# swishersnaaake/sexy-raytracer

Hardware: AMD Instinct MI355X
Metric: Msamples/s (WxHxspp/s), 720p masterchief @5k spp (higher is better)
Workload: dtype f32; 1 GPU; masterchief_720p_5000spp; scene=masterchief, width=1280, height=720, spp=5000, max_bounce=4, seed=1, spp_chunks=625, tree=reference, traversal=faithful (bvh.h order), parallelism=tiles8x8 interleaved over 1 rank(s), 1 gather (none)

## Files before the change

sexy-raytracer_amd/csrc/srt_api.cpp:

```cpp

#include <hip/hip_runtime.h>

#include <algorithm>
#include <cstdarg>
#include <cstdio>
#include <cstdlib>
#include <cstring>
#include <string>
#include <vector>

#include "srt_context.h"
#include "srt_launch.h"
#include "srt_thread.h"

int fail(SrtContext* ctx, const char* fmt, ...) {
  char buf[512];
  va_list ap;
  va_start(ap, fmt);
  vsnprintf(buf, sizeof buf, fmt, ap);
  va_end(ap);
  if (ctx) ctx->error = buf;
  fprintf(stderr, "srt_hip: %s\n", buf);
  return 1;
}

int wfCheck(SrtContext* ctx) {
  if (ctx->dWfError && *(volatile int32_t*)ctx->dWfError != 0) {
// ... 39 lines not shown
    {"node_burst", "SRT_NODE_BURST", &Tunables::nodeBurst, -1},
    {"ploc_radius", "SRT_PLOC_RADIUS", &Tunables::plocRadius, 64},
    {"fast_div", "SRT_FAST_DIV", &Tunables::fastDiv, 1},
    {"prim_again_min", "SRT_PRIM_AGAIN_MIN", &Tunables::primAgainMin, 4},
    {"keep_eighths", "SRT_KEEP_EIGHTHS", &Tunables::keepEighths, -1},
    {"chunk_scratch_mb", "SRT_CHUNK_SCRATCH_MB", &Tunables::chunkScratchMb, 12288},
    {"lds_tree", "SRT_LDS_TREE", &Tunables::ldsTree, 1},
    {"wavefront", "SRT_WAVEFRONT", &Tunables::wavefront, 256},
    {"wf_pool", "SRT_WF_POOL", &Tunables::wfPool, 2048},
    {"wf_swap_min", "SRT_WF_SWAP_MIN", &Tunables::wfSwapMin, 0},
    {"wf_swap_big", "SRT_WF_SWAP_BIG", &Tunables::wfSwapBig, 32},
    {"wf_profile", "SRT_WF_PROFILE", &Tunables::wfProfile, 0},
    {"wf_hybrid", "SRT_WF_HYBRID", &Tunables::wfHybrid, 1},
    {"wf_resident_max", "SRT_WF_RESIDENT_MAX", &Tunables::wfResidentMax, 0},
    {"wf_far_rounds", "SRT_WF_FAR_ROUNDS", &Tunables::wfFarRounds, 0},
    {"denoise_lds_step", "SRT_DENOISE_LDS_STEP", &Tunables::denoiseLdsStep, 4},
    {"tri_cert", "SRT_TRI_CERT", &Tunables::triCert, 1},
};

float triWMaxFor(const SrtContext* ctx) { return ctx->tun.triCert ? SRT_TRI_W_MAX : 0.0f; }

}

int checkSceneReady(SrtContext* ctx, const char* what) {
  if (!ctx->upload.haveScene) return fail(ctx, "%s: no scene uploaded", what);
  if (ctx->upload.geometryDirty) return fail(ctx, "%s: geometry was updated; call srtRefitScene before anything traverses the scene", what);
  return 0;
}

int buildDeviceTrees(SrtContext* ctx) {
// ... 19 lines not shown
  return 0;
}

static int srtUploadSceneImpl(SrtContext* ctx, const SrtSceneDesc* d) {
  if (!ctx || !d) return 1;
  HIP_OK(ctx, hipSetDevice(ctx->device));
  ctx->upload = Upload();
  ctx->temporalValid = false;
  std::string err = validateScene(d);
  HostScene h;
  if (err.empty()) err = flattenScene(d, SceneOptions{ctx->tun.wfHybrid, ctx->tun.wfResidentMax, ctx->tun.fastDiv}, h);
  if (!err.empty()) return fail(ctx, "%s", err.c_str());

  DevScene& s = ctx->upload.scene;
  if (!h.nodeThread.empty() && uploadVec(ctx, h.nodeThread, &s.nodeThread)) return 1;
  if (!h.nodesWf.empty() && (uploadVec(ctx, h.nodesWf, &s.nodesWf) || uploadVec(ctx, h.worldWf, &s.worldWf) || uploadVec(ctx, h.primSecond, &s.primSecond))) return 1;
  if (uploadVec(ctx, h.primClass, &s.primClass, 16) || uploadVec(ctx, h.nodeAxis, &s.nodeAxis, 64) || uploadVec(ctx, h.nodes, &s.nodes) ||
      uploadVec(ctx, h.triTest, &s.triTest) || uploadVec(ctx, h.triFast, &s.triFast) || uploadVec(ctx, h.triShade, &s.triShade) || uploadVec(ctx, h.spheres, &s.spheres) ||
      uploadVec(ctx, h.triPrimId, &s.triPrimId) || uploadVec(ctx, h.sphPrimId, &s.sphPrimId) || uploadVec(ctx, h.world, &s.world) ||
      uploadVec(ctx, h.materials, &s.materials) || uploadVec(ctx, h.shadeRecs, &s.shadeRecs) || uploadVec(ctx, h.textures, &s.textures) ||
      uploadVec(ctx, h.texels, &s.texels, 64))
    return 1;
  s.wfResident = h.wfResident;
  s.numPrimClass = (int32_t)h.primClass.size();
  s.numWorld = (int32_t)h.world.size();
  s.stackDepth = h.stackDepth;
  s.numNodes = (int32_t)(h.nodes.size() / 2);
  s.numTris = d->numTriangles;
  s.numSpheres = d->numSpheres;
  s.numMaterials = d->numMaterials;
// ... 226 lines not shown

int srtTestHybridRecords(const float* nodes8, int32_t numNodes, const int32_t* world, int32_t numWorld, int32_t numTriangles, int32_t numSpheres,
                         int32_t cap, float* outNodes8, int32_t* outWorld, int32_t* outSecond) {
  if (!nodes8 || !world || !outNodes8 || !outWorld || !outSecond || numNodes < 0 || numWorld < 0 || cap < 0) return -1;
  std::vector<float4> nodes(2 * (size_t)numNodes), wf;
  if (numNodes) memcpy(nodes.data(), nodes8, nodes.size() * sizeof(float4));
  std::vector<int32_t> w, second;
  const int32_t resident = srtHybridRecords(nodes, std::vector<int32_t>(world, world + numWorld), numTriangles, numSpheres, (size_t)cap, wf, w, second);
  if (resident <= 0) return 0;
  memcpy(outNodes8, wf.data(), wf.size() * sizeof(float4));
  memcpy(outWorld, w.data(), w.size() * sizeof(int32_t));
  memcpy(outSecond, second.data(), second.size() * sizeof(int32_t));
  return resident;
}

int srtTestGetTreeAux(SrtContext* ctx, int32_t item, uint8_t* outAxis, float* outPairs16, int32_t capacity, int32_t* count) {
  if (!ctx || !count) return 1;
  if (!ctx->upload.haveScene) return fail(ctx, "srtTestGetTreeAux: no scene uploaded");
  if (item < 0 || item >= (int32_t)ctx->upload.itemNodes.size()) return fail(ctx, "srtTestGetTreeAux: item %d out of range", item);
  HIP_OK(ctx, hipSetDevice(ctx->device));
  int32_t ref = 0;
  HIP_OK(ctx, hipMemcpy(&ref, ctx->upload.scene.world + item, sizeof ref, hipMemcpyDeviceToHost));
  if (ref < 0) return fail(ctx, "srtTestGetTreeAux: item %d is not a tree", item);
  const auto dt = std::find_if(ctx->upload.deviceBuilds.begin(), ctx->upload.deviceBuilds.end(), [&](const DeviceBuild& b) { return b.item == item; });
  const int32_t base = SRT_NODE_INDEX(ref), n = dt != ctx->upload.deviceBuilds.end() ? dt->count : (int32_t)ctx->upload.itemNodes[item].size();
  if (base + n > ctx->upload.scene.numNodes) return fail(ctx, "srtTestGetTreeAux: item %d lies outside the node array", item);
  *count = n;
  if (!outAxis && !outPairs16) return 0;
  if (capacity < n) return fail(ctx, "srtTestGetTreeAux: capacity %d < %d", capacity, n);
  if (outAxis) HIP_OK(ctx, hipMemcpy(outAxis, ctx->upload.scene.nodeAxis + base, (size_t)n, hipMemcpyDeviceToHost));
// ... 124 lines not shown
```

sexy-raytracer_amd/csrc/srt_context.h:

```cpp
#pragma once
#include <hip/hip_runtime.h>

#include <algorithm>
#include <cstring>
#include <exception>
#include <string>
#include <vector>

#include "srt_buffer.h"
#include "srt_device.h"
#include "srt_scene.h"

struct Tunables {
  int tileBlock, unitTiles, queues;
  int shadeMin, primMin, hitMin, fuseMin, nodeBurst;
  int plocRadius, fastDiv;
  int chunkScratchMb;
  int primAgainMin;
  int keepEighths;
  int ldsTree;
  int wavefront, wfPool, wfSwapMin, wfSwapBig, wfProfile;
  int wfHybrid, wfResidentMax, wfFarRounds;
  int denoiseLdsStep;
  int triCert;
};

struct Upload {
  std::vector<DeviceBuffer> sceneBuffers;
  DevScene scene{};
  bool haveScene = false;
  std::vector<std::vector<SrtBvhNode>> itemNodes;
  std::vector<DeviceBuild> deviceBuilds;
  std::vector<DeviceBuffer> buildRefs;
  int plocRadius = 0;
  int hostStackDepth = 0, hostBvhDepth = 0;
  std::vector<int32_t> hostTriPrimId, hostSphPrimId;
  int bvhDepth = 0;
  struct Tree {
    int32_t item, base, count;
    float time0, time1;
    bool deviceBuilt;
  };
  std::vector<Tree> trees;
  std::vector<int32_t> hostTriDevIndex, hostWfIndex;
  std::vector<uint8_t> itemBoxesStale;
  DeviceBuffer triDevIndex, wfIndex, refitUp, refitArrived;
  bool refitTables = false;
  bool refitLinksStale = false;
  bool geometryDirty = false;
  float pairTime0 = 0, pairTime1 = 0;
  int32_t fastDivOption = 0;
  DeviceBuffer prevTriTest, prevSpheres;
  bool haveSnapshot = false;
  bool epochSnapshot = false;
};

struct SrtContext {
  int device = 0;
  std::string error;
  Tunables tun{};
  hipDeviceProp_t prop;
// ... 117 lines not shown
```

sexy-raytracer_amd/csrc/srt_device.h:

```cpp
#ifndef SRT_DEVICE_H
#define SRT_DEVICE_H

#include <stdint.h>

#include "../../include/srt_hip.h"
#include "../../include/srt_hip_test.h"

#define SRT_REF_DONE ((int32_t)0x80000000)
#define SRT_NODE_REF(index) ((int32_t)(index) << 5)
#define SRT_NODE_INDEX(ref) ((int32_t)(ref) >> 5)
#define SRT_MAX_NODES (1 << 25)
#define SRT_MAX_QUEUES 64
#define SRT_BLOCK 256
#define SRT_BLOCK_TREE 1024
#define SRT_MAT_INDEX_MASK 0x00ffffff
#define SRT_MAT_TYPE_SHIFT 24
#define SRT_MAT_TEXTURED 4
#define SRT_MAT_FLAGS_SHIFT 28

struct DevMaterial {
  int32_t type;
  int32_t albedoTex, normalTex, metallicTex, roughnessTex;
  float albedo[4];
  float metalness, roughness;
// ... 27 lines not shown
  const int32_t* primSecond;
  int32_t wfResident;
  const int32_t* triPrimId;
  const int32_t* sphPrimId;
  const int32_t* world;
  int32_t numWorld;
  int32_t stackDepth;
  int32_t numNodes, numTris, numSpheres;
  int32_t fastDivScene;
  const DevMaterial* materials;
  const uint4* shadeRecs;
  int32_t numMaterials;
  const DevTexture* textures;
  const uint8_t* texels;
  int32_t texelBytes;
};

struct DevCamera {
  float origin[3], lleft[3], horizontal[3], vertical[3], hor[3], vert[3];
  float lensRadius, time0, time1;
};

struct SrtFixedAccum {
  long long r, g, b;
  uint32_t flags;
  uint32_t pad;
};

struct RenderArgs {
  DevScene scene;
// ... 205 lines not shown
```

sexy-raytracer_amd/csrc/srt_path.h:

```cpp
#ifndef SRT_PATH_H
#define SRT_PATH_H

#include <hip/hip_runtime.h>

#include <type_traits>
#include <stdint.h>

#include "srt_device.h"
#include "srt_slab.h"
#include "srt_tri_hit.h"

#define SRT_TREE_WAVES_PER_SIMD 4
#ifndef SRT_NODE_UNROLL
#define SRT_NODE_UNROLL 4
#endif
#ifndef SRT_NODE_UNROLL_CLOSEST
#define SRT_NODE_UNROLL_CLOSEST 4
#endif
#ifndef SRT_PRIM_ROUNDS
#define SRT_PRIM_ROUNDS 2
#endif
#ifndef SRT_RENDER_WAVES_PER_SIMD
#define SRT_RENDER_WAVES_PER_SIMD 5
#endif
// ... 118 lines not shown
  tMin = fmaxf(fminf(a, b), tMin);
  tMax = fminf(fmaxf(a, b), tMax);
  return !(tMax <= tMin);
}

__device__ __forceinline__ SrtSlab3 slab3(V3 v) { return SrtSlab3{v.x, v.y, v.z}; }
template <bool UNIFORM_TMIN>
__device__ __forceinline__ bool boxHitApprox(float4 n0, float4 n1, V3 r1, V3 m, float tolAbs, float tMin, float tMax,
                                             bool& undecided) {
  return srtSlabVerdict<UNIFORM_TMIN, false>(srtSlabEndsMinMax(n0, n1, slab3(r1), slab3(m)), tolAbs, tMin, tMax, undecided);
}
template <bool UNIFORM_TMIN>
__device__ __forceinline__ bool boxHitSign(float4 n0, float4 n1, V3 rp, V3 rq, V3 m, float tolAbs, float tMin, float tMax,
                                           bool& undecided) {
  return srtSlabVerdict<UNIFORM_TMIN, true>(srtSlabEndsSign(n0, n1, slab3(rp), slab3(rq), slab3(m)), tolAbs, tMin, tMax, undecided);
}
__device__ __forceinline__ bool boxMaybeHit(float4 lo, float4 hi, V3 r1, V3 m, float tolAbs, float tMin, float tMax, float& tEnter) {
  return srtSlabMaybe<false>(srtSlabEndsMinMax(lo, hi, slab3(r1), slab3(m)), tolAbs, tMin, tMax, tEnter);
}
__device__ __forceinline__ void slabSetup(const V3& o, const V3& r1, bool certified, V3& m, float& tolAbs) {
  SrtSlab3 mm;
  srtSlabSetup(slab3(o), slab3(r1), certified, mm, tolAbs);
  m = mk(mm.x, mm.y, mm.z);
}
__device__ __forceinline__ void slabSetupSign(const V3& o, const V3& r1, bool certified, V3& rp, V3& rq, V3& m, float& tolAbs) {
  SrtSlab3 p, q, mm;
  srtSlabSignSetup(slab3(o), slab3(r1), certified, p, q, mm, tolAbs);
  rp = mk(p.x, p.y, p.z);
  rq = mk(q.x, q.y, q.z);
  m = mk(mm.x, mm.y, mm.z);
// ... 498 lines not shown
```

sexy-raytracer_amd/csrc/srt_refit_host.cpp:

```cpp

#include <hip/hip_runtime.h>

#include <algorithm>
#include <cstdint>
#include <cstring>
#include <vector>

#include "srt_context.h"
#include "srt_launch.h"

namespace {

int checkUpdate(SrtContext* ctx, const char* what, int32_t first, int32_t count, int32_t have, const void* in, size_t align) {
  if (!ctx->upload.haveScene) return fail(ctx, "%s: no scene uploaded", what);
  if (first < 0 || count < 0 || (int64_t)first + count > have)
    return fail(ctx, "%s: range [%d, %d + %d) lies outside the scene's %d records", what, first, first, count, have);
  if (count == 0) return 2;
  if (!in) return fail(ctx, "%s: null records", what);
  if ((uintptr_t)in % align) return fail(ctx, "%s: records must be aligned to %zu bytes", what, align);
  return 0;
}

int triangleTable(SrtContext* ctx, const int32_t** out) {
  *out = nullptr;
// ... 92 lines not shown
    if (!ctx->upload.refitTables) {
      HIP_OK(ctx, ctx->upload.refitUp.reserve((size_t)n * sizeof(int32_t)));
      HIP_OK(ctx, ctx->upload.refitArrived.reserve((size_t)n * sizeof(int32_t)));
      HIP_OK(ctx, ctx->refitFlag.reserve(16));
      if (s.nodesWf) {
        if (ctx->upload.hostWfIndex.size() != (size_t)n) return fail(ctx, "%s: the hybrid records have no renumbering", what);
        HIP_OK(ctx, ctx->upload.wfIndex.reserve((size_t)n * sizeof(int32_t)));
        HIP_OK(ctx, hipMemcpy(ctx->upload.wfIndex.get(), ctx->upload.hostWfIndex.data(), (size_t)n * sizeof(int32_t), hipMemcpyHostToDevice));
      }
      ctx->upload.refitTables = ctx->upload.refitLinksStale = true;
    }
    if (ctx->upload.refitLinksStale) {
      const int e = srt_launch_refit_links(s.nodes, n, ctx->upload.refitUp.get<int32_t>(), stream);
      if (e) return fail(ctx, "%s: launch failed: %s", what, hipGetErrorString((hipError_t)e));
      ctx->upload.refitLinksStale = false;
    }
    HIP_OK(ctx, hipMemsetAsync(ctx->upload.refitArrived.get(), 0, (size_t)n * sizeof(int32_t), stream));
    HIP_OK(ctx, hipMemsetAsync(ctx->refitFlag.get(), 0, 16, stream));
    int e = 0;
    for (const Upload::Tree& t : ctx->upload.trees) {
      if (t.base < 0 || t.count < 1 || t.base + t.count > n) return fail(ctx, "%s: world item %d lies outside the node array", what, t.item);
      e = srt_launch_refit_nodes(&s, t.base, t.count, t.time0, t.time1, ctx->upload.refitUp.get<const int32_t>(), ctx->upload.refitArrived.get<int32_t>(),
                                 ctx->refitFlag.get<int32_t>(), t.deviceBuilt ? 1 : 0, stream);
      if (e) break;
    }
    if (!e) e = srt_launch_refit_derived(&s, s.nodesWf ? ctx->upload.wfIndex.get<const int32_t>() : nullptr, ctx->refitFlag.get<int32_t>(), stream);
    if (!e) e = srt_pair_nodes_async(&s, ctx->upload.pairTime0, ctx->upload.pairTime1, const_cast<float4*>(s.nodes2), stream);
    if (e) return fail(ctx, "%s: launch failed: %s", what, hipGetErrorString((hipError_t)e));
    HIP_OK(ctx, hipMemcpyAsync(&flag, ctx->refitFlag.get(), sizeof flag, hipMemcpyDeviceToHost, stream));
  }
  if (hipStreamSynchronize(stream) != hipSuccess) return fail(ctx, "%s: kernel failed: %s", what, hipGetErrorString(hipGetLastError()));
  ctx->upload.scene.fastDivScene = (flag & 3) == 0 ? ctx->upload.fastDivOption : 0;
  ctx->upload.scene.boxOrderedScene = (flag & 4) == 0 ? 1 : 0;
  if (ctx->motionTracking) {
    if (ctx->temporalRefits < 2) ctx->temporalRefits++;
    ctx->upload.epochSnapshot = false;
  } else {
    ctx->temporalValid = false;
  }
// ... 63 lines not shown
```

sexy-raytracer_amd/csrc/srt_render.cpp:

```cpp

#include <hip/hip_runtime.h>

#include <algorithm>
#include <cstring>
#include <vector>

#include "srt_context.h"
#include "srt_launch.h"

namespace {

size_t ldsBytesFor(const SrtContext* ctx, int maxBounce, int stackDepth) {
  return (size_t)(stackDepth + 2 + 3 * maxBounce + 3) * SRT_BLOCK * sizeof(int32_t) + 4 * sizeof(int32_t);
}

float chunkFixLimit(int32_t chunks) {
  int pow2 = 1;
  while (pow2 < chunks) pow2 *= 2;
  return 0x1p26f / (float)pow2;
}

}

extern "C" {
// ... 163 lines not shown
      if (!scratchPath) return fail(ctx, "render: cannot allocate %zu B for the pixel sums", need);
      scratchPath = false;
      HIP_OK(ctx, ctx->chunkScratch.reserve(planes * tilePixels * sizeof(SrtFixedAccum)));
    }
    if (scratchPath) {
      a.out = ctx->chunkScratch.get<float4>();
      a.chunkStride = (int32_t)tilePixels;
      if (moments) a.mout = a.out + tilePixels * a.sppChunks;
    } else {
      a.fix = ctx->chunkScratch.get<SrtFixedAccum>();
      if (moments) a.mfix = a.fix + tilePixels;
      HIP_OK(ctx, hipMemsetAsync(a.fix, 0, planes * tilePixels * sizeof(SrtFixedAccum), stream));
    }
  }
  const RenderPlan plan = renderPlan(ctx, p, moments, dList ? listTiles : -1);
  if (plan.lds > 160 * 1024) return fail(ctx, "render: BVH depth %d needs %zu B of LDS per workgroup", ctx->upload.scene.stackDepth, plan.lds);
  const RenderKernel kernel = plan.form >= 3 ? srt_render_wf_kernel_for(&plan) : srt_render_kernel_for(&plan);
  if (plan.lds > 64 * 1024)
    HIP_OK(ctx, hipFuncSetAttribute(reinterpret_cast<const void*>(kernel), hipFuncAttributeMaxDynamicSharedMemorySize, (int)plan.lds));
  int perCU = 1;
  if (plan.form < 3 && (hipOccupancyMaxActiveBlocksPerMultiprocessor(&perCU, kernel, plan.block, plan.lds) != hipSuccess || perCU < 1)) perCU = 1;
  const int wgItems = SRT_TILE_PIXELS * (plan.block / 64);
  int grid = std::min(ctx->prop.multiProcessorCount * perCU, (a.numWork + wgItems - 1) / wgItems);
  if (grid < 1) grid = 1;
  if (plan.form >= 3) {
    const int64_t itemsPerGroup = ((int64_t)a.numWork + grid - 1) / grid;
    const int wfPoolSize = (int)std::max<int64_t>(64, std::min<int64_t>(plan.wfRingCap, itemsPerGroup + 63));
    HIP_OK(ctx, ctx->wfPool.reserve((size_t)grid * wfPoolSize * 128));
    const int hiLevels = std::max(0, p->maxBounce - 4);
    HIP_OK(ctx, ctx->wfAttHi.reserve(std::max<size_t>(16, (size_t)grid * 3 * hiLevels * wfPoolSize * sizeof(float))));
// ... 541 lines not shown
```

sexy-raytracer_amd/csrc/srt_scene.cpp:

```cpp

#include "srt_scene.h"

#include <algorithm>
#include <cmath>
#include <cstdarg>
#include <cstdio>
#include <cstring>
#include <limits>
#include <random>

#include "srt_thread.h"

namespace {

std::mt19937& hostGenerator() {
  static std::mt19937 generator;
  return generator;
}
float hostRandomFloat() {
  static std::uniform_real_distribution<float> distribution(0.0f, 1.0f);
  return distribution(hostGenerator());
}
int hostRandomInt(int lo, int hi) {
  float a = (float)lo, b = (float)(hi + 1);
  return static_cast<int>(a + (b - a) * hostRandomFloat());
// ... 188 lines not shown
                    &h.triFast[SRT_TRI_FAST_SLOTS * (size_t)i]);
  }
  h.spheres.resize((size_t)d->numSpheres * 3);
  for (int i = 0; i < d->numSpheres; ++i) {
    const SrtSphereIn& s = d->spheres[i];
    sphereRecords(vec3(s.center0), vec3(s.center1), s.time0, s.time1, s.radius, s.material, &h.spheres[3 * (size_t)i]);
  }
  std::vector<int32_t> triDevIndex;
  auto devRef = [&](int32_t listRef) -> int32_t {
    const SrtPrimRef& p = d->prims[~listRef];
    if (p.type == SRT_PRIM_SPHERE) return ~((p.index << 1) | 1);
    return ~((triDevIndex.empty() ? p.index : triDevIndex[p.index]) << 1);
  };

  h.itemNodes.resize(d->numWorld);
  for (int w = 0; w < d->numWorld; ++w) {
    const SrtWorldItem& it = d->world[w];
    if (it.kind == SRT_WORLD_PRIM) {
      h.world.push_back(devRef(~it.first));
      continue;
    }
    if (!it.nodes && (it.builder == SRT_BUILDER_LBVH || it.builder == SRT_BUILDER_PLOC)) {
      int32_t base = (int32_t)(h.nodes.size() / 2), cnt = std::max(it.count - 1, 1);
      h.nodes.resize(h.nodes.size() + 2 * (size_t)cnt, make_float4(0, 0, 0, 0));
      h.nodeAxis.resize(h.nodeAxis.size() + cnt, 3);
      h.deviceBuilds.push_back(DeviceBuild{w, base, cnt, it.builder, it.time0, it.time1, {}});
      h.world.push_back(SRT_NODE_REF(base));
      continue;
    }
    Builder b;
    buildItem(d, it, b);
    int32_t base = (int32_t)(h.nodes.size() / 2);
// ... 180 lines not shown
    }
  }
  h.fastDivScene = certified ? o.fastDiv : 0;
  h.boxOrderedScene = ordered ? 1 : 0;
  if (h.deviceBuilds.empty() && !h.nodes.empty()) {
    srtThreadLinks16(h.nodes, h.world, d->numTriangles, d->numSpheres, h.nodeThread);
    if (o.wfHybrid > 0) {
      const size_t n = h.nodes.size() / 2;
      const size_t fits = (160 * 1024 - 64 * sizeof(int32_t) - 20 * 2048) / 32;
      const size_t fitsWhole = (160 * 1024 - 64 * sizeof(int32_t) - 18 * 1024) / 32;
      const size_t cap = o.wfResidentMax > 0 ? std::min<size_t>(fits, (size_t)o.wfResidentMax) : fits;
      if (n > (o.wfResidentMax > 0 ? cap : fitsWhole))
        h.wfResident = srtHybridRecords(h.nodes, h.world, d->numTriangles, d->numSpheres, cap, h.nodesWf, h.worldWf, h.primSecond, &h.wfIndex);
      if (h.nodesWf.empty()) h.wfIndex.clear();
    }
  }
  auto classOf = [&](float word, bool sphere) -> uint8_t {
    const int32_t bits = bitsAs<int32_t>(&word);
    const int type = (bits >> SRT_MAT_TYPE_SHIFT) & 3, flags = (bits >> SRT_MAT_FLAGS_SHIFT) & 3;
    if (type != SRT_MAT_PBR) return 2;
    if (!sphere) return 0;
    return flags ? 2 : 1;
  };
  h.triDevIndex.swap(triDevIndex);
  h.primClass.assign((size_t)2 * std::max(d->numTriangles, d->numSpheres) + 2, 2);
  for (int i = 0; i < d->numTriangles; ++i) h.primClass[(size_t)i << 1] = classOf(h.triShade[4 * (size_t)i + 3].w, false);
  for (int i = 0; i < d->numSpheres; ++i) h.primClass[((size_t)i << 1) | 1] = classOf(h.spheres[3 * (size_t)i + 1].w, true);
  return std::string();
}

// ... 34 lines not shown
```

sexy-raytracer_amd/csrc/srt_scene.h:

```cpp
#pragma once
#include <hip/hip_runtime.h>

#include <cstdint>
#include <string>
#include <vector>

#include "srt_device.h"
#include "srt_records.h"

struct BuildNode {
  Box box;
  int32_t left, right;
  uint8_t axis = 3;
};

struct Builder {
  const SrtSceneDesc* d;
  float time0, time1;
  std::vector<float> sortKey;
  std::vector<int32_t> objects;
  std::vector<BuildNode> nodes;
  int maxPending = 0;

  Box childBox(int32_t ref) const;
// ... 25 lines not shown
  float time0, time1;
};

struct HostScene {
  std::vector<float4> nodes;
  std::vector<uint8_t> nodeAxis;
  std::vector<int32_t> world;
  std::vector<float4> triTest, triShade, triFast, spheres;
  std::vector<int32_t> triPrimId, sphPrimId;
  std::vector<DevMaterial> materials;
  std::vector<DevTexture> textures;
  std::vector<uint8_t> texels;
  std::vector<uint4> shadeRecs;
  std::vector<uint8_t> primClass;
  std::vector<int32_t> nodeThread;
  std::vector<float4> nodesWf;
  std::vector<int32_t> worldWf, primSecond;
  int32_t wfResident = 0;
  std::vector<std::vector<SrtBvhNode>> itemNodes;
  std::vector<DeviceBuild> deviceBuilds;
  std::vector<HostTree> hostTrees;
  std::vector<int32_t> triDevIndex;
  std::vector<int32_t> wfIndex;
  int stackDepth = 0, bvhDepth = 0;
  int32_t fastDivScene = 0;
  int32_t boxOrderedScene = 0;
};

std::string flattenScene(const SrtSceneDesc* d, const SceneOptions& o, HostScene& out);
```

sexy-raytracer_amd/csrc/srt_slab.h:

```cpp
#pragma once
#include <hip/hip_runtime.h>
#include <math.h>

#include "srt_device.h"

struct SrtSlab3 {
  float x, y, z;
};

#define SRT_SLAB_FN SRT_HD __forceinline__
#if defined(__HIP_DEVICE_COMPILE__)
#define SRT_SLAB_ASM2(op, a, b)          \
  float r;                               \
  asm(op " %0, %1, %2" : "=v"(r) : "v"(a), "v"(b)); \
  return r
#define SRT_SLAB_ASM3(op, a, b, c)       \
  float r;                               \
  asm(op " %0, %1, %2, %3" : "=v"(r) : "v"(a), "v"(b), "v"(c)); \
  return r
#endif
SRT_SLAB_FN float srtSlabMin(float a, float b) {
#if defined(__HIP_DEVICE_COMPILE__)
  SRT_SLAB_ASM2("v_min_f32", a, b);
#else
// ... 78 lines not shown
  return srtSlabMin3(srtSlabMax(e.a.x, e.b.x), srtSlabMax(e.a.y, e.b.y), srtSlabMax(e.a.z, e.b.z));
}

#define SRT_SLAB_EPS 0x1p-21f

template <bool UNIFORM_TMIN, bool ORDERED>
SRT_SLAB_FN bool srtSlabVerdict(const SrtSlabEnds& e, float tolAbs, float tMin, float tMax, bool& undecided) {
  const float lo = srtSlabNear<ORDERED>(e);
  tMin = UNIFORM_TMIN ? srtSlabMaxUniform(lo, tMin) : srtSlabMax(lo, tMin);
  tMax = srtSlabMin(srtSlabFar<ORDERED>(e), tMax);
  const float diff = tMax - tMin;
  const float tol = __builtin_fmaf(SRT_SLAB_EPS, fabsf(tMax) + fabsf(tMin), tolAbs);
  undecided = !(fabsf(diff) > tol);
  return diff > tol;
}
template <bool ORDERED>
SRT_SLAB_FN bool srtSlabMaybe(const SrtSlabEnds& e, float tolAbs, float tMin, float tMax, float& tEnter) {
  const float t0 = srtSlabMax(srtSlabNear<ORDERED>(e), tMin);
  const float t1 = srtSlabMin(srtSlabFar<ORDERED>(e), tMax);
  const float tol = __builtin_fmaf(SRT_SLAB_EPS, fabsf(t1) + fabsf(t0), tolAbs);
  tEnter = t0;
  return !(t1 - t0 < -tol);
}
```

sexy-raytracer_amd/csrc/srt_wavefront.hip:

```cpp
#include "srt_path.h"
#include "srt_launch.h"
#include "srt_wf_links.h"
#include "srt_wf_rings.h"

#define WF_BLOCK 1024
#define WF_SET_OF(mask) std::integral_constant<uint32_t, (mask)>()
#define WF_CTX_BYTES 128
#define WF_CTL_LIVE 28
#define WF_CTL_ABORT 29
#define WF_CTL_WORDS 64
#define WF_PEND_MISS 0
#define WF_PEND_TERMINAL 2

namespace {
enum { W_NODE = 0, W_PRIM = 1, W_SWAP = 2, W_SERVE = 3 };

__device__ __forceinline__ void bufStore4(Rsrc r, int off, float4 v) {
  u32x4 u;
  u.x = __float_as_uint(v.x); u.y = __float_as_uint(v.y); u.z = __float_as_uint(v.z); u.w = __float_as_uint(v.w);
  __builtin_amdgcn_raw_buffer_store_b128(u, r, off, 0, 0);
}
__device__ __forceinline__ void bufStore1(Rsrc r, int off, uint32_t v) { __builtin_amdgcn_raw_buffer_store_b32(v, r, off, 0, 0); }
typedef float f32x4 __attribute__((ext_vector_type(4)));
typedef __attribute__((address_space(3))) const f32x4 LdsVec4;
// ... 10 lines not shown
  typedef typename std::conditional<HYBRID, int32_t, uint16_t>::type PrimSlot;
  extern __shared__ int32_t lds[];
  const DevScene& sc = a.scene;
  char* const ldsTree = reinterpret_cast<char*>(lds);
  const int resident = HYBRID ? sc.wfResident : sc.numNodes;
  const int treeBytes = resident * 32;
  int32_t* const ctl = reinterpret_cast<int32_t*>(ldsTree + treeBytes);
  const int RCAP = a.wfRingCap, POOL = a.wfPoolSize;
  uint16_t* const ringSlots = reinterpret_cast<uint16_t*>(ctl + WF_CTL_WORDS);
  float* const hitT = reinterpret_cast<float*>(ringSlots + WF_RINGS * RCAP);
  PrimSlot* const hitPrim = reinterpret_cast<PrimSlot*>(hitT + POOL);
  const int lane = threadIdx.x & 63;
  const unsigned long long laneBelow = (1ull << lane) - 1ull;
  const uint64_t seedMixed = mix64(a.seed);
  const V3 background = ld3(a.background);
  const Rsrc rsNodes = makeRsrc(HYBRID ? sc.nodesWf : sc.nodes, sc.numNodes * 32);
  const Rsrc rsTris = makeRsrc(sc.triTest, HYBRID ? sc.numTris * 48 : 0);
  const Rsrc rsFast = makeRsrc(sc.triFast, HYBRID ? 0 : sc.numTris * 64);
  const Rsrc rsSpheres = makeRsrc(sc.spheres, sc.numSpheres * 48);
  const Rsrc rsTexels = makeRsrc(sc.texels, sc.texelBytes);
  const Rsrc rsClass = makeRsrc(sc.primClass, sc.numPrimClass);
  const Rsrc rsSecond = makeRsrc(sc.primSecond, HYBRID ? sc.numPrimClass * 4 : 0);
  const Rsrc rsPool = makeRsrc(a.wfPool + (size_t)blockIdx.x * POOL * WF_CTX_BYTES, POOL * WF_CTX_BYTES);
  const int hiLevels = a.maxBounce > 4 ? a.maxBounce - 4 : 0;
  const Rsrc rsAttHi = makeRsrc(a.wfAttHi + (size_t)blockIdx.x * 3 * hiLevels * POOL, 3 * hiLevels * POOL * 4);
  const bool singleRoot = SINGLE || sc.numWorld == 1;
  auto worldRef = [&](int k) {
    if (HYBRID) return sc.worldWf[k];
    return srtWfRootWord(sc.world[k]);
  };
  const SrtWfRingGeom ringGeom = {a.wfRingCap, a.wfRingShift, a.wfRingMul3};

  {
    float4* dst = reinterpret_cast<float4*>(ldsTree);
    for (int i = threadIdx.x; i < resident * 2; i += WF_BLOCK) {
      float4 v = bufLoad4(rsNodes, 16 * i);
      if (!HYBRID) {
        const int32_t thread = sc.nodeThread[i >> 1];
        v.w = __int_as_float((i & 1) ? srtWfMissWord(thread) : srtWfHitWord(__float_as_int(v.w), thread));
      }
      dst[i] = v;
    }
    for (int i = threadIdx.x; i < WF_CTL_WORDS; i += WF_BLOCK) ctl[i] = 0;
    for (int i = threadIdx.x; i < WF_RINGS * RCAP; i += WF_BLOCK) ringSlots[i] = 0;
    __syncthreads();
    for (int id = threadIdx.x; id < POOL; id += WF_BLOCK) ringSlots[WF_RING_NEWITEM * RCAP + id] = (uint16_t)(id + 1);
    if (threadIdx.x == 0) {
      ctl[WF_CTL_TAIL(WF_RING_NEWITEM)] = POOL;
      ctl[WF_CTL_LIVE] = POOL;
    }
    if (threadIdx.x < 16) ctl[threadIdx.x] = (int)(blockIdx.x % (unsigned)a.numQueues);
    __syncthreads();
  }
// ... 162 lines not shown
      }
      return nNodes;
  };
  auto nodeBurst = [&](int nNodes) -> int {
      const int keep = (nNodes * a.keepEighths) >> 3;
      int budget = a.nodeBurst, left;
      auto visit = [&](const float4 n0, const float4 n1) {
        bool undecided;
        bool hitBox = SIGNFORM ? boxHitSign<true>(n0, n1, rp, rq, negOR, slabTol, a.tMin, closest, undecided)
                               : boxHitApprox<true>(n0, n1, rp, negOR, slabTol, a.tMin, closest, undecided);
        if (PROFILE) {
          const unsigned long long mu = __ballot(undecided);
          pLanes[8] += __popcll(mu);
          pLanes[7] += mu != 0 ? 1 : 0;
        }
        if (undecided) hitBox = boxHit(n0, n1, ray, a.tMin, closest);
        if constexpr (COUNT) {
          cnt[2]++;
          if (hitBox) cnt[3]++;
        }
        link = __float_as_int(n1.w);
        cur = hitBox ? __float_as_int(n0.w) : (HYBRID ? link >> 2 : link);
        if (!SINGLE && !singleRoot && cur == DONE && ++w < sc.numWorld) {
          cur = worldRef(w);
          link = DONE_PAIR;
        }
      };
      auto nodeVisit = [&](bool mine) {
        const bool here = HYBRID ? mine && (uint32_t)cur < (uint32_t)resident : cur >= 0;
        if (PROFILE) {
          pRuns[0]++;
// ... 501 lines not shown
```

sexy-raytracer_amd/hipdev.py:

```python
import ctypes as C
import os

import numpy as np

from . import abi

_HERE = os.path.dirname(os.path.abspath(__file__))
LIB_PATH = os.path.join(_HERE, "csrc", "libsrt_hip.so")
if os.environ.get("SRT_HIP_LIB"):
    LIB_PATH = os.path.abspath(os.environ["SRT_HIP_LIB"])

if not os.path.exists(LIB_PATH):
    raise ImportError("HIP extension not built: %s is missing (run __graft_entry__.build() or "
                      "`make -C sexy-raytracer_amd/csrc`)" % LIB_PATH)

try:
    import torch
except ImportError:
    pass

lib = C.CDLL(LIB_PATH)

EXPORTS = ["srtCreate", "srtDestroy", "srtLastError", "srtMakeCamera", "srtHostRandomFloat", "srtHostRandomReset",
           "srtUploadScene", "srtSetCamera", "srtBuildBvh", "srtGetBvh", "srtGetBvhDepth", "srtNumTiles", "srtNumLocalTiles", "srtDefaultSppChunks", "srtPlanSppChunks",
# ... 4 lines not shown
           "srtRenderTilesMoments", "srtRenderImageMoments", "srtDenoiseMoments", "srtRenderDenoisedImageMoments",
           "srtRenderAdaptive", "srtRenderAdaptiveImage",
           "srtTemporalAccumulate", "srtRenderTemporalFrame", "srtTemporalReset",
           "srtTemporalReproject", "srtRenderTemporalAdaptive", "srtRenderTemporalAdaptiveFrame",
           "srtRenderFeatureTileList", "srtRenderAdaptiveGuided", "srtRenderAdaptiveDenoisedImage",
           "srtRenderTemporalAdaptiveGuided", "srtRenderTemporalAdaptiveGuidedFrame",
           "srtUpdateTriangles", "srtUpdateSpheres", "srtUpdateTrianglesDevice", "srtUpdateSpheresDevice", "srtRefitScene",
           "srtRebuildScene", "srtGetTreeCost",
           "srtSetMotionTracking", "srtRenderMotionTiles", "srtRenderMotionImage", "srtTemporalAccumulateMotion",
           "srtTemporalReprojectMotion",
           "srtCommGetUniqueId", "srtCommInit", "srtGatherTiles", "srtRenderImageRanks", "srtCommDestroy",
           "srtLastKernelMs", "srtGetStats", "srtDeviceInfo"]
TEST_EXPORTS = ["srtSetTunable", "srtGetTunable", "srtGetShadeProfile", "srtGetWfProfile", "srtGetLaunchInfo", "srtRenderAov",
                "srtScatterRaysForm", "srtTestThreadLinks16", "srtTestHybridRecords", "srtTestGetTreeAux", "srtTestChunkSum",
                "srtTestDenoiseScratch", "srtTestGetTriUndecided", "srtTestGetTriFast", "srtTestTriFastRecord", "srtTestGetSlabScene",
                "srtTestRefinedRcp", "srtTestSlabVisit"]

_vp = C.c_void_p
lib.srtCreate.argtypes = [C.c_int, C.POINTER(_vp)]
lib.srtDestroy.argtypes = [_vp]
lib.srtLastError.argtypes = [_vp]
lib.srtLastError.restype = C.c_char_p
lib.srtMakeCamera.argtypes = [C.POINTER(abi.SrtCameraParams), C.POINTER(abi.SrtCamera)]
lib.srtHostRandomFloat.restype = C.c_float
lib.srtHostRandomReset.restype = None
lib.srtUploadScene.argtypes = [_vp, C.POINTER(abi.SrtSceneDesc)]
lib.srtSetCamera.argtypes = [_vp, C.POINTER(abi.SrtCamera)]
lib.srtBuildBvh.argtypes = [C.POINTER(abi.SrtSceneDesc), C.c_int32, _vp, C.c_int32, C.POINTER(C.c_int32),
                            C.POINTER(C.c_int32)]
lib.srtGetBvh.argtypes = [_vp, C.c_int32, _vp, C.c_int32, C.POINTER(C.c_int32)]
lib.srtGetBvhDepth.argtypes = [_vp, C.POINTER(C.c_int32)]
# ... 87 lines not shown
lib.srtGetWfProfile.argtypes = [_vp, _vp]
lib.srtGetLaunchInfo.argtypes = [_vp, _vp]
lib.srtTestThreadLinks16.argtypes = [_vp, C.c_int32, _vp, C.c_int32, C.c_int32, C.c_int32, _vp]
lib.srtTestHybridRecords.argtypes = [_vp, C.c_int32, _vp, C.c_int32, C.c_int32, C.c_int32, C.c_int32, _vp, _vp, _vp]
lib.srtTestThreadLinks16.restype = lib.srtTestHybridRecords.restype = C.c_int32
lib.srtTestGetTreeAux.argtypes = [_vp, C.c_int32, C.POINTER(C.c_uint8), C.POINTER(C.c_float), C.c_int32, C.POINTER(C.c_int32)]
if hasattr(lib, "srtTestGetTriUndecided"):
    lib.srtTestGetTriUndecided.argtypes = [_vp, C.POINTER(C.c_uint64)]
    lib.srtTestGetTriFast.argtypes = [_vp, _vp, C.c_int32, C.POINTER(C.c_int32)]
    lib.srtTestTriFastRecord.argtypes = [_vp, _vp]
if hasattr(lib, "srtTestGetSlabScene"):
    lib.srtTestGetSlabScene.argtypes = [_vp, C.POINTER(C.c_int32)]
if hasattr(lib, "srtTestRefinedRcp"):
    lib.srtTestRefinedRcp.argtypes = [_vp, C.c_int64, C.c_int64, C.POINTER(C.c_uint64)]
    lib.srtTestSlabVisit.argtypes = [_vp, C.POINTER(C.c_float), C.c_int32, C.c_float, C.c_int32, C.POINTER(C.c_float)]
lib.srtRenderAov.argtypes = [_vp, C.POINTER(abi.SrtRenderParams), C.c_int32, _vp]
lib.srtLastKernelMs.argtypes = [_vp, C.POINTER(C.c_float)]
lib.srtGetStats.argtypes = [_vp, C.POINTER(abi.SrtStats)]
lib.srtDeviceInfo.argtypes = [_vp, C.c_char_p, C.c_int32, C.POINTER(C.c_int32), C.POINTER(C.c_int32)]


class SrtError(RuntimeError):
    pass


def make_camera(params):
    cam = abi.SrtCamera()
    if lib.srtMakeCamera(C.byref(params), C.byref(cam)):
        raise SrtError("srtMakeCamera failed")
    return cam

# ... 585 lines not shown
        return int(out.value)

    def tri_fast_records(self):
        n = C.c_int32(0)
        self._check(lib.srtTestGetTriFast(self.h, None, 0, C.byref(n)))
        out = np.zeros((n.value, 16), np.float32)
        if n.value:
            self._check(lib.srtTestGetTriFast(self.h, out.ctypes.data, n.value, C.byref(n)))
        return out

    def slab_scene(self):
        out = (C.c_int32 * 2)()
        self._check(lib.srtTestGetSlabScene(self.h, out))
        return int(out[0]), int(out[1])

    def refined_rcp_test(self, first_bits, count):
        out = (C.c_uint64 * 2)()
        self._check(lib.srtTestRefinedRcp(self.h, int(first_bits), int(count), out))
        return float(np.array([out[0]], np.uint64).view(np.float64)[0]), np.array([out[1]], np.uint32).view(np.float32)[0]

    def slab_visit_test(self, cases, t_min, certified_scene=1):
        cases = np.ascontiguousarray(cases, np.float32)
        if cases.ndim != 2 or cases.shape[1] != 13:
            raise ValueError("cases must be (n, 13)")
        out = np.zeros((len(cases), 8), np.float32)
        fp = C.POINTER(C.c_float)
        self._check(lib.srtTestSlabVisit(self.h, cases.ctypes.data_as(fp), len(cases), float(t_min), int(certified_scene), out.ctypes.data_as(fp)))
        return out

    def set_tunable(self, name, value):
# ... 59 lines not shown
```

Measured before the change: 5990 Msamples/s.

## Rebuild BVH topology with SAH split over leaf order for wavefront traversal

Adds a host-side regrouping pass that keeps each tree's leaf order but re-chooses the internal split points with a surface-area cost, producing a second node array and thread links. The wavefront non-hybrid kernel loads this tree into LDS and traverses it, using a new exact slab test with a gate for zero-direction axes on internal nodes. The aim is fewer box visits per ray through tighter internal bounds. In exchange it costs extra scene memory, extra refit work, and a changed traversal order whose result must match the faithful order.

```diff
diff --git a/sexy-raytracer_amd/csrc/srt_api.cpp b/sexy-raytracer_amd/csrc/srt_api.cpp
--- a/sexy-raytracer_amd/csrc/srt_api.cpp
+++ b/sexy-raytracer_amd/csrc/srt_api.cpp
@@ -11,6 +11,7 @@
 
 #include "srt_context.h"
 #include "srt_launch.h"
+#include "srt_regroup.h"
 #include "srt_thread.h"
 
 int fail(SrtContext* ctx, const char* fmt, ...) {
@@ -80,6 +81,7 @@
     {"wf_hybrid", "SRT_WF_HYBRID", &Tunables::wfHybrid, 1},
     {"wf_resident_max", "SRT_WF_RESIDENT_MAX", &Tunables::wfResidentMax, 0},
     {"wf_far_rounds", "SRT_WF_FAR_ROUNDS", &Tunables::wfFarRounds, 0},
+    {"wf_regroup", "SRT_WF_REGROUP", &Tunables::wfRegroup, 1},
     {"denoise_lds_step", "SRT_DENOISE_LDS_STEP", &Tunables::denoiseLdsStep, 4},
     {"tri_cert", "SRT_TRI_CERT", &Tunables::triCert, 1},
 };
@@ -129,6 +131,7 @@
 
   DevScene& s = ctx->upload.scene;
   if (!h.nodeThread.empty() && uploadVec(ctx, h.nodeThread, &s.nodeThread)) return 1;
+  if (!h.nodesRg.empty() && (uploadVec(ctx, h.nodesRg, &s.nodesRg) || uploadVec(ctx, h.nodeThreadRg, &s.nodeThreadRg))) return 1;
   if (!h.nodesWf.empty() && (uploadVec(ctx, h.nodesWf, &s.nodesWf) || uploadVec(ctx, h.worldWf, &s.worldWf) || uploadVec(ctx, h.primSecond, &s.primSecond))) return 1;
   if (uploadVec(ctx, h.primClass, &s.primClass, 16) || uploadVec(ctx, h.nodeAxis, &s.nodeAxis, 64) || uploadVec(ctx, h.nodes, &s.nodes) ||
       uploadVec(ctx, h.triTest, &s.triTest) || uploadVec(ctx, h.triFast, &s.triFast) || uploadVec(ctx, h.triShade, &s.triShade) || uploadVec(ctx, h.spheres, &s.spheres) ||
@@ -385,6 +388,28 @@
   return resident;
 }
 
+int srtTestRegroup(const float* nodes8, int32_t numNodes, const int32_t* world, int32_t numWorld, float* outNodes8) {
+  if (!nodes8 || !world || !outNodes8 || numNodes < 0 || numWorld < 0) return -1;
+  std::vector<float4> nodes(2 * (size_t)numNodes), out;
+  if (numNodes) memcpy(nodes.data(), nodes8, nodes.size() * sizeof(float4));
+  if (!srtRegroupNodes(nodes, std::vector<int32_t>(world, world + numWorld), out)) return 0;
+  if (numNodes) memcpy(outNodes8, out.data(), out.size() * sizeof(float4));
+  return 1;
+}
+int srtTestGetRegroup(SrtContext* ctx, float* outNodes8, int32_t* outLinks, int32_t capacity, int32_t* count) {
+  if (!ctx || !count) return 1;
+  if (!ctx->upload.haveScene) return fail(ctx, "srtTestGetRegroup: no scene uploaded");
+  const DevScene& s = ctx->upload.scene;
+  *count = s.nodesRg ? s.numNodes : 0;
+  if (!s.nodesRg || (!outNodes8 && !outLinks)) return 0;
+  if (capacity < s.numNodes) return fail(ctx, "srtTestGetRegroup: capacity %d < %d", capacity, s.numNodes);
+  HIP_OK(ctx, hipSetDevice(ctx->device));
+  HIP_OK(ctx, hipDeviceSynchronize());
+  if (outNodes8) HIP_OK(ctx, hipMemcpy(outNodes8, s.nodesRg, (size_t)s.numNodes * 32, hipMemcpyDeviceToHost));
+  if (outLinks) HIP_OK(ctx, hipMemcpy(outLinks, s.nodeThreadRg, (size_t)s.numNodes * sizeof(int32_t), hipMemcpyDeviceToHost));
+  return 0;
+}
+
 int srtTestGetTreeAux(SrtContext* ctx, int32_t item, uint8_t* outAxis, float* outPairs16, int32_t capacity, int32_t* count) {
   if (!ctx || !count) return 1;
   if (!ctx->upload.haveScene) return fail(ctx, "srtTestGetTreeAux: no scene uploaded");
diff --git a/sexy-raytracer_amd/csrc/srt_context.h b/sexy-raytracer_amd/csrc/srt_context.h
--- a/sexy-raytracer_amd/csrc/srt_context.h
+++ b/sexy-raytracer_amd/csrc/srt_context.h
@@ -21,6 +21,7 @@
   int ldsTree;
   int wavefront, wfPool, wfSwapMin, wfSwapBig, wfProfile;
   int wfHybrid, wfResidentMax, wfFarRounds;
+  int wfRegroup;
   int denoiseLdsStep;
   int triCert;
 };
@@ -45,6 +46,7 @@
   std::vector<int32_t> hostTriDevIndex, hostWfIndex;
   std::vector<uint8_t> itemBoxesStale;
   DeviceBuffer triDevIndex, wfIndex, refitUp, refitArrived;
+  DeviceBuffer refitUpRg;
   bool refitTables = false;
   bool refitLinksStale = false;
   bool geometryDirty = false;
diff --git a/sexy-raytracer_amd/csrc/srt_device.h b/sexy-raytracer_amd/csrc/srt_device.h
--- a/sexy-raytracer_amd/csrc/srt_device.h
+++ b/sexy-raytracer_amd/csrc/srt_device.h
@@ -65,6 +65,8 @@
   const DevTexture* textures;
   const uint8_t* texels;
   int32_t texelBytes;
+  const float4* nodesRg;
+  const int32_t* nodeThreadRg;
 };
 
 struct DevCamera {
diff --git a/sexy-raytracer_amd/csrc/srt_path.h b/sexy-raytracer_amd/csrc/srt_path.h
--- a/sexy-raytracer_amd/csrc/srt_path.h
+++ b/sexy-raytracer_amd/csrc/srt_path.h
@@ -156,6 +156,9 @@
 __device__ __forceinline__ bool boxHitSign(float4 n0, float4 n1, V3 rp, V3 rq, V3 m, float tolAbs, float tMin, float tMax,
                                            bool& undecided) {
   return srtSlabVerdict<UNIFORM_TMIN, true>(srtSlabEndsSign(n0, n1, slab3(rp), slab3(rq), slab3(m)), tolAbs, tMin, tMax, undecided);
+}
+__device__ __forceinline__ bool boxHitOrGate(float4 n0, float4 n1, const Ray& r, float tMin, float tMax, bool gate) {
+  return srtSlabExactOrGate(n0, n1, slab3(r.o), slab3(r.d), tMin, tMax, gate);
 }
 __device__ __forceinline__ bool boxMaybeHit(float4 lo, float4 hi, V3 r1, V3 m, float tolAbs, float tMin, float tMax, float& tEnter) {
   return srtSlabMaybe<false>(srtSlabEndsMinMax(lo, hi, slab3(r1), slab3(m)), tolAbs, tMin, tMax, tEnter);
diff --git a/sexy-raytracer_amd/csrc/srt_refit_host.cpp b/sexy-raytracer_amd/csrc/srt_refit_host.cpp
--- a/sexy-raytracer_amd/csrc/srt_refit_host.cpp
+++ b/sexy-raytracer_amd/csrc/srt_refit_host.cpp
@@ -130,6 +130,11 @@
       const int e = srt_launch_refit_links(s.nodes, n, ctx->upload.refitUp.get<int32_t>(), stream);
       if (e) return fail(ctx, "%s: launch failed: %s", what, hipGetErrorString((hipError_t)e));
       ctx->upload.refitLinksStale = false;
+      if (s.nodesRg) {
+        HIP_OK(ctx, ctx->upload.refitUpRg.reserve((size_t)n * sizeof(int32_t)));
+        const int eRg = srt_launch_refit_links(s.nodesRg, n, ctx->upload.refitUpRg.get<int32_t>(), stream);
+        if (eRg) return fail(ctx, "%s: launch failed: %s", what, hipGetErrorString((hipError_t)eRg));
+      }
     }
     HIP_OK(ctx, hipMemsetAsync(ctx->upload.refitArrived.get(), 0, (size_t)n * sizeof(int32_t), stream));
     HIP_OK(ctx, hipMemsetAsync(ctx->refitFlag.get(), 0, 16, stream));
@@ -139,6 +144,16 @@
       e = srt_launch_refit_nodes(&s, t.base, t.count, t.time0, t.time1, ctx->upload.refitUp.get<const int32_t>(), ctx->upload.refitArrived.get<int32_t>(),
                                  ctx->refitFlag.get<int32_t>(), t.deviceBuilt ? 1 : 0, stream);
       if (e) break;
+    }
+    if (!e && s.nodesRg) {
+      DevScene rg = s;
+      rg.nodes = s.nodesRg;
+      e = (int)hipMemsetAsync(ctx->upload.refitArrived.get(), 0, (size_t)n * sizeof(int32_t), stream);
+      for (const Upload::Tree& t : ctx->upload.trees) {
+        if (e) break;
+        e = srt_launch_refit_nodes(&rg, t.base, t.count, t.time0, t.time1, ctx->upload.refitUpRg.get<const int32_t>(),
+                                   ctx->upload.refitArrived.get<int32_t>(), ctx->refitFlag.get<int32_t>(), 0, stream);
+      }
     }
     if (!e) e = srt_launch_refit_derived(&s, s.nodesWf ? ctx->upload.wfIndex.get<const int32_t>() : nullptr, ctx->refitFlag.get<int32_t>(), stream);
     if (!e) e = srt_pair_nodes_async(&s, ctx->upload.pairTime0, ctx->upload.pairTime1, const_cast<float4*>(s.nodes2), stream);
diff --git a/sexy-raytracer_amd/csrc/srt_regroup.h b/sexy-raytracer_amd/csrc/srt_regroup.h
--- /dev/null
+++ b/sexy-raytracer_amd/csrc/srt_regroup.h
@@ -0,0 +1,117 @@
+#pragma once
+#include <hip/hip_runtime.h>
+
+#include <cassert>
+#include <cmath>
+#include <cstdint>
+#include <cstring>
+#include <vector>
+
+#include "srt_device.h"
+#include "srt_records.h"
+
+namespace srt_regroup_detail {
+inline int32_t refOf(const std::vector<float4>& nodes, size_t slot) {
+  int32_t r;
+  memcpy(&r, &nodes[slot].w, 4);
+  return r;
+}
+inline Box boxOfNode(const std::vector<float4>& nodes, size_t i) {
+  return Box{{nodes[2 * i].x, nodes[2 * i].y, nodes[2 * i].z}, {nodes[2 * i + 1].x, nodes[2 * i + 1].y, nodes[2 * i + 1].z}};
+}
+inline double halfArea(const Box& b) {
+  const double x = (double)b.mx[0] - b.mn[0], y = (double)b.mx[1] - b.mn[1], z = (double)b.mx[2] - b.mn[2];
+  return x * y + y * z + z * x;
+}
+inline Box unite(const Box& a, const Box& b) {
+  const Box r = surrounding(a, b);
+  for (int k = 0; k < 3; ++k) {
+    assert(memcmp(&r.mn[k], &a.mn[k], 4) == 0 || memcmp(&r.mn[k], &b.mn[k], 4) == 0);
+    assert(memcmp(&r.mx[k], &a.mx[k], 4) == 0 || memcmp(&r.mx[k], &b.mx[k], 4) == 0);
+  }
+  return r;
+}
+}
+
+inline bool srtRegroupNodes(const std::vector<float4>& nodes, const std::vector<int32_t>& world, std::vector<float4>& out) {
+  using namespace srt_regroup_detail;
+  const size_t n = nodes.size() / 2;
+  out = nodes;
+  std::vector<uint8_t> seen(n, 0);
+  struct Range {
+    int32_t me, lo, hi;
+  };
+  std::vector<int32_t> leaves, todo;
+  std::vector<Box> leafBox, prefix, suffix;
+  std::vector<Range> ranges;
+  for (int32_t wr : world) {
+    if (wr < 0) continue;
+    const int32_t root = SRT_NODE_INDEX(wr);
+    leaves.clear();
+    todo.assign(1, root);
+    int32_t count = 0, last = root;
+    while (!todo.empty()) {
+      const int32_t i = todo.back();
+      todo.pop_back();
+      if (i < 0 || (size_t)i >= n || seen[i]) return out.clear(), false;
+      seen[i] = 1;
+      count++;
+      last = i > last ? i : last;
+      const int32_t l = refOf(nodes, 2 * (size_t)i), r = refOf(nodes, 2 * (size_t)i + 1);
+      if ((l >= 0) != (r >= 0)) return out.clear(), false;
+      if (l >= 0) {
+        todo.push_back(SRT_NODE_INDEX(r));
+        todo.push_back(SRT_NODE_INDEX(l));
+      } else {
+        leaves.push_back(i);
+      }
+    }
+    if (last - root + 1 != count || (size_t)count != 2 * leaves.size() - 1) return out.clear(), false;
+    const int32_t numLeaves = (int32_t)leaves.size();
+    leafBox.resize(numLeaves);
+    for (int32_t k = 0; k < numLeaves; ++k) leafBox[k] = boxOfNode(nodes, (size_t)leaves[k]);
+    prefix.resize(numLeaves);
+    suffix.resize(numLeaves);
+    ranges.assign(1, Range{root, 0, numLeaves});
+    while (!ranges.empty()) {
+      const Range g = ranges.back();
+      ranges.pop_back();
+      const int32_t span = g.hi - g.lo;
+      if (span == 1) {
+        out[2 * (size_t)g.me] = nodes[2 * (size_t)leaves[g.lo]];
+        out[2 * (size_t)g.me + 1] = nodes[2 * (size_t)leaves[g.lo] + 1];
+        continue;
+      }
+      prefix[g.lo] = leafBox[g.lo];
+      for (int32_t k = g.lo + 1; k < g.hi; ++k) prefix[k] = unite(prefix[k - 1], leafBox[k]);
+      suffix[g.hi - 1] = leafBox[g.hi - 1];
+      for (int32_t k = g.hi - 2; k >= g.lo; --k) suffix[k] = unite(leafBox[k], suffix[k + 1]);
+      int32_t bestK = 1;
+      double best = 0.0;
+      for (int32_t k = 1; k < span; ++k) {
+        const double cost = halfArea(prefix[g.lo + k - 1]) * k + halfArea(suffix[g.lo + k]) * (span - k);
+        if (k == 1 || cost < best) {
+          best = cost;
+          bestK = k;
+        }
+      }
+      const int32_t left = g.me + 1, right = g.me + 2 * bestK;
+      const int32_t lRef = SRT_NODE_REF(left), rRef = SRT_NODE_REF(right);
+      float lBits, rBits;
+      memcpy(&lBits, &lRef, 4);
+      memcpy(&rBits, &rRef, 4);
+      out[2 * (size_t)g.me] = make_float4(0.0f, 0.0f, 0.0f, lBits);
+      out[2 * (size_t)g.me + 1] = make_float4(0.0f, 0.0f, 0.0f, rBits);
+      ranges.push_back(Range{right, g.lo + bestK, g.hi});
+      ranges.push_back(Range{left, g.lo, g.lo + bestK});
+    }
+    for (int32_t i = root + count - 1; i >= root; --i) {
+      const int32_t l = refOf(out, 2 * (size_t)i), r = refOf(out, 2 * (size_t)i + 1);
+      if (l < 0) continue;
+      const Box b = unite(boxOfNode(out, (size_t)SRT_NODE_INDEX(l)), boxOfNode(out, (size_t)SRT_NODE_INDEX(r)));
+      out[2 * (size_t)i].x = b.mn[0], out[2 * (size_t)i].y = b.mn[1], out[2 * (size_t)i].z = b.mn[2];
+      out[2 * (size_t)i + 1].x = b.mx[0], out[2 * (size_t)i + 1].y = b.mx[1], out[2 * (size_t)i + 1].z = b.mx[2];
+    }
+  }
+  return true;
+}
diff --git a/sexy-raytracer_amd/csrc/srt_render.cpp b/sexy-raytracer_amd/csrc/srt_render.cpp
--- a/sexy-raytracer_amd/csrc/srt_render.cpp
+++ b/sexy-raytracer_amd/csrc/srt_render.cpp
@@ -201,6 +201,7 @@
     }
   }
   const RenderPlan plan = renderPlan(ctx, p, moments, dList ? listTiles : -1);
+  if (plan.form != 3 || plan.count || ctx->tun.wfRegroup <= 0 || !a.scene.boxOrderedScene) a.scene.nodesRg = nullptr, a.scene.nodeThreadRg = nullptr;
   if (plan.lds > 160 * 1024) return fail(ctx, "render: BVH depth %d needs %zu B of LDS per workgroup", ctx->upload.scene.stackDepth, plan.lds);
   const RenderKernel kernel = plan.form >= 3 ? srt_render_wf_kernel_for(&plan) : srt_render_kernel_for(&plan);
   if (plan.lds > 64 * 1024)
diff --git a/sexy-raytracer_amd/csrc/srt_scene.cpp b/sexy-raytracer_amd/csrc/srt_scene.cpp
--- a/sexy-raytracer_amd/csrc/srt_scene.cpp
+++ b/sexy-raytracer_amd/csrc/srt_scene.cpp
@@ -9,6 +9,7 @@
 #include <limits>
 #include <random>
 
+#include "srt_regroup.h"
 #include "srt_thread.h"
 
 namespace {
@@ -227,8 +228,10 @@
   };
 
   h.itemNodes.resize(d->numWorld);
+  bool adopted = false;
   for (int w = 0; w < d->numWorld; ++w) {
     const SrtWorldItem& it = d->world[w];
+    adopted = adopted || (it.kind == SRT_WORLD_BVH && it.nodes);
     if (it.kind == SRT_WORLD_PRIM) {
       h.world.push_back(devRef(~it.first));
       continue;
@@ -439,6 +442,19 @@
         h.wfResident = srtHybridRecords(h.nodes, h.world, d->numTriangles, d->numSpheres, cap, h.nodesWf, h.worldWf, h.primSecond, &h.wfIndex);
       if (h.nodesWf.empty()) h.wfIndex.clear();
     }
+    const size_t fitsWholeTree = (160 * 1024 - 64 * sizeof(int32_t) - 18 * 1024) / 32;
+    if (!h.nodeThread.empty() && h.nodesWf.empty() && !adopted && ordered && h.nodes.size() / 2 <= fitsWholeTree &&
+        srtRegroupNodes(h.nodes, h.world, h.nodesRg)) {
+      srtThreadLinks16(h.nodesRg, h.world, d->numTriangles, d->numSpheres, h.nodeThreadRg);
+      bool same = !h.nodeThreadRg.empty();
+      for (const float4& v : h.nodesRg) same = same && (!certified || (fastDivOperand(v.x) && fastDivOperand(v.y) && fastDivOperand(v.z)));
+      for (size_t i = 0; same && i + 1 < h.nodesRg.size(); i += 2)
+        same = srtBoxOrdered(Box{{h.nodesRg[i].x, h.nodesRg[i].y, h.nodesRg[i].z}, {h.nodesRg[i + 1].x, h.nodesRg[i + 1].y, h.nodesRg[i + 1].z}});
+      if (!same) {
+        h.nodesRg.clear();
+        h.nodeThreadRg.clear();
+      }
+    }
   }
   auto classOf = [&](float word, bool sphere) -> uint8_t {
     const int32_t bits = bitsAs<int32_t>(&word);
diff --git a/sexy-raytracer_amd/csrc/srt_scene.h b/sexy-raytracer_amd/csrc/srt_scene.h
--- a/sexy-raytracer_amd/csrc/srt_scene.h
+++ b/sexy-raytracer_amd/csrc/srt_scene.h
@@ -63,6 +63,8 @@
   std::vector<uint4> shadeRecs;
   std::vector<uint8_t> primClass;
   std::vector<int32_t> nodeThread;
+  std::vector<float4> nodesRg;
+  std::vector<int32_t> nodeThreadRg;
   std::vector<float4> nodesWf;
   std::vector<int32_t> worldWf, primSecond;
   int32_t wfResident = 0;
diff --git a/sexy-raytracer_amd/csrc/srt_slab.h b/sexy-raytracer_amd/csrc/srt_slab.h
--- a/sexy-raytracer_amd/csrc/srt_slab.h
+++ b/sexy-raytracer_amd/csrc/srt_slab.h
@@ -116,6 +116,25 @@
   undecided = !(fabsf(diff) > tol);
   return diff > tol;
 }
+SRT_SLAB_FN void srtSlabExactAxis(float n0, float n1, float o, float d, bool gate, float& tMin, float& tMax, bool& inside) {
+  const float a = (n0 - o) / d, b = (n1 - o) / d;
+  const float lo = fmaxf(fminf(a, b), tMin), hi = fminf(fmaxf(a, b), tMax);
+  const bool closed = gate & (d == 0.0f);
+  tMin = closed ? tMin : lo;
+  tMax = closed ? tMax : hi;
+  inside = inside & !(closed & ((o < n0) | (o > n1)));
+}
+SRT_SLAB_FN bool srtSlabExactOrGate(float4 n0, float4 n1, SrtSlab3 o, SrtSlab3 d, float tMin, float tMax, bool gate) {
+  bool inside = true;
+  srtSlabExactAxis(n0.x, n1.x, o.x, d.x, gate, tMin, tMax, inside);
+  srtSlabExactAxis(n0.y, n1.y, o.y, d.y, gate, tMin, tMax, inside);
+  srtSlabExactAxis(n0.z, n1.z, o.z, d.z, gate, tMin, tMax, inside);
+  return inside & !(tMax <= tMin);
+}
+SRT_SLAB_FN bool srtSlabGateExact(float4 n0, float4 n1, SrtSlab3 o, SrtSlab3 d, float tMin, float tMax) {
+  return srtSlabExactOrGate(n0, n1, o, d, tMin, tMax, true);
+}
+
 template <bool ORDERED>
 SRT_SLAB_FN bool srtSlabMaybe(const SrtSlabEnds& e, float tolAbs, float tMin, float tMax, float& tEnter) {
   const float t0 = srtSlabMax(srtSlabNear<ORDERED>(e), tMin);
diff --git a/sexy-raytracer_amd/csrc/srt_wavefront.hip b/sexy-raytracer_amd/csrc/srt_wavefront.hip
--- a/sexy-raytracer_amd/csrc/srt_wavefront.hip
+++ b/sexy-raytracer_amd/csrc/srt_wavefront.hip
@@ -48,7 +48,8 @@
   const unsigned long long laneBelow = (1ull << lane) - 1ull;
   const uint64_t seedMixed = mix64(a.seed);
   const V3 background = ld3(a.background);
-  const Rsrc rsNodes = makeRsrc(HYBRID ? sc.nodesWf : sc.nodes, sc.numNodes * 32);
+  const bool regroup = !HYBRID && !COUNT && sc.nodesRg != nullptr;
+  const Rsrc rsNodes = makeRsrc(HYBRID ? sc.nodesWf : (regroup ? sc.nodesRg : sc.nodes), sc.numNodes * 32);
   const Rsrc rsTris = makeRsrc(sc.triTest, HYBRID ? sc.numTris * 48 : 0);
   const Rsrc rsFast = makeRsrc(sc.triFast, HYBRID ? 0 : sc.numTris * 64);
   const Rsrc rsSpheres = makeRsrc(sc.spheres, sc.numSpheres * 48);
@@ -67,10 +68,11 @@
 
   {
     float4* dst = reinterpret_cast<float4*>(ldsTree);
+    const int32_t* const threads = regroup ? sc.nodeThreadRg : sc.nodeThread;
     for (int i = threadIdx.x; i < resident * 2; i += WF_BLOCK) {
       float4 v = bufLoad4(rsNodes, 16 * i);
       if (!HYBRID) {
-        const int32_t thread = sc.nodeThread[i >> 1];
+        const int32_t thread = threads[i >> 1];
         v.w = __int_as_float((i & 1) ? srtWfMissWord(thread) : srtWfHitWord(__float_as_int(v.w), thread));
       }
       dst[i] = v;
@@ -263,7 +265,11 @@
           pLanes[8] += __popcll(mu);
           pLanes[7] += mu != 0 ? 1 : 0;
         }
-        if (undecided) hitBox = boxHit(n0, n1, ray, a.tMin, closest);
+        if constexpr (HYBRID || COUNT) {
+          if (undecided) hitBox = boxHit(n0, n1, ray, a.tMin, closest);
+        } else {
+          if (undecided) hitBox = boxHitOrGate(n0, n1, ray, a.tMin, closest, regroup & (__float_as_int(n0.w) >= 0));
+        }
         if constexpr (COUNT) {
           cnt[2]++;
           if (hitBox) cnt[3]++;
diff --git a/sexy-raytracer_amd/hipdev.py b/sexy-raytracer_amd/hipdev.py
--- a/sexy-raytracer_amd/hipdev.py
+++ b/sexy-raytracer_amd/hipdev.py
@@ -42,7 +42,7 @@
 TEST_EXPORTS = ["srtSetTunable", "srtGetTunable", "srtGetShadeProfile", "srtGetWfProfile", "srtGetLaunchInfo", "srtRenderAov",
                 "srtScatterRaysForm", "srtTestThreadLinks16", "srtTestHybridRecords", "srtTestGetTreeAux", "srtTestChunkSum",
                 "srtTestDenoiseScratch", "srtTestGetTriUndecided", "srtTestGetTriFast", "srtTestTriFastRecord", "srtTestGetSlabScene",
-                "srtTestRefinedRcp", "srtTestSlabVisit"]
+                "srtTestRefinedRcp", "srtTestSlabVisit", "srtTestRegroup", "srtTestGetRegroup"]
 
 _vp = C.c_void_p
 lib.srtCreate.argtypes = [C.c_int, C.POINTER(_vp)]
@@ -160,7 +160,11 @@
 if hasattr(lib, "srtTestRefinedRcp"):
     lib.srtTestRefinedRcp.argtypes = [_vp, C.c_int64, C.c_int64, C.POINTER(C.c_uint64)]
     lib.srtTestSlabVisit.argtypes = [_vp, C.POINTER(C.c_float), C.c_int32, C.c_float, C.c_int32, C.POINTER(C.c_float)]
-lib.srtRenderAov.argtypes = [_vp, C.POINTER(abi.SrtRenderParams), C.c_int32, _vp]
+if hasattr(lib, "srtTestRegroup"):
+    lib.srtTestRegroup.argtypes = [_vp, C.c_int32, _vp, C.c_int32, _vp]
+    lib.srtTestRegroup.restype = C.c_int32
+    lib.srtTestGetRegroup.argtypes = [_vp, _vp, _vp, C.c_int32, C.POINTER(C.c_int32)]
+lib.srtRenderAov.argtypes =[_vp, C.POINTER(abi.SrtRenderParams), C.c_int32, _vp]
 lib.srtLastKernelMs.argtypes = [_vp, C.POINTER(C.c_float)]
 lib.srtGetStats.argtypes = [_vp, C.POINTER(abi.SrtStats)]
 lib.srtDeviceInfo.argtypes = [_vp, C.c_char_p, C.c_int32, C.POINTER(C.c_int32), C.POINTER(C.c_int32)]
@@ -776,6 +780,15 @@
         self._check(lib.srtTestGetSlabScene(self.h, out))
         return int(out[0]), int(out[1])
 
+    def regroup(self):
+        n = C.c_int32(0)
+        self._check(lib.srtTestGetRegroup(self.h, None, None, 0, C.byref(n)))
+        if n.value == 0:
+            return None
+        nodes, links = np.zeros((n.value, 8), np.float32), np.zeros(n.value, np.int32)
+        self._check(lib.srtTestGetRegroup(self.h, nodes.ctypes.data, links.ctypes.data, n.value, C.byref(n)))
+        return nodes, links
+
     def refined_rcp_test(self, first_bits, count):
         out = (C.c_uint64 * 2)()
         self._check(lib.srtTestRefinedRcp(self.h, int(first_bits), int(count), out))
```

Result: faster. 6651 Msamples/s, median of 6 (+11.0%).
